# orybkin/video-gcp

Hardware: AMD Instinct MI355X
Metric: predicted frames/sec, 64x64x3 seq_len=80 gcp_tree (posterior forward + all loss terms, model(inputs) and model.loss() of train.py:157-159, batch-stat BatchNorm) (higher is better)
Workload: dtype f32 (encoder / decoder convs and the tree GEMMs from 512 rows: split-f16 MFMA with f32 accumulate, f32-equivalent; everything else exact f32 MFMA)

## Files before the change

### video-gcp_amd/csrc/aux.hip

```cpp
#include "common.h"

namespace {

template <bool GAUSS>
__global__ void aux_sample_indices_kernel(const long long* __restrict__ end_ind, const float* __restrict__ u, const int B,
                                          const int temp_dist, long long* __restrict__ t0, long long* __restrict__ t1,
                                          long long* __restrict__ cs, long long* __restrict__ ce) {
    const int b = blockIdx.x * blockDim.x + threadIdx.x;
    if (b >= B) return;
    const long long e = end_ind[b];
    const double ed = (double)e;
    auto uni = [&](int k) { const double v = (double)u[k * B + b]; return GAUSS ? 0.5 * erfc(-v * 0.70710678118654752440) : v; };
    long long a = (long long)floor(uni(0) * (ed - temp_dist + 1));
    a = max(min(a, e - temp_dist), 0ll);
    long long d = (long long)floor(uni(1) * temp_dist);
    d = min(d, (long long)temp_dist - 1);
    long long s = (long long)floor(uni(2) * ed);
    s = min(s, e - 1);
    long long w = (long long)floor(uni(3) * (ed - (double)s));
    w = min(w, e - s - 1);
    t0[b] = a;
    t1[b] = min(a + 1 + d, max(e, 0ll));
    cs[b] = s;
    ce[b] = s + 1 + w;
}

__global__ void aux_index_rows_kernel(const long long* __restrict__ t0, const long long* __restrict__ t1,
                                      const long long* __restrict__ cs, const long long* __restrict__ ce, const int B, const int T,
                                      const int Wd, int* __restrict__ rows) {
    const int b = blockIdx.x * blockDim.x + threadIdx.x;
    if (b >= B) return;
    rows[b] = b * T + (int)t0[b];
    rows[B + b] = b * Wd + (int)t1[b];
    rows[2 * B + b] = b * Wd + (int)cs[b];
    rows[3 * B + b] = b * Wd + (int)ce[b];
}

template <int VEC>
__global__ void __launch_bounds__(256) path_cost_rows_kernel(const float* __restrict__ x, const long long* __restrict__ cs,
                                                             const long long* __restrict__ ce, const int T, const int rows,
                                                             const int row_len, float* __restrict__ partial) {
    const int lane = threadIdx.x & 63;
    const int row = blockIdx.x * 4 + (threadIdx.x >> 6);
    const int b = blockIdx.y;
    if (row >= rows) return;
    const int s = (int)cs[b], e = (int)ce[b];
    const size_t frame = (size_t)rows * row_len;
    const float* p = x + ((size_t)b * T + s) * frame + (size_t)row * row_len;
    float acc = 0.f;
    for (int t = s; t < e; ++t) {
        float d2 = 0.f;
        for (int c = lane * VEC; c < row_len; c += 64 * VEC) {
#pragma unroll
            for (int v = 0; v < VEC; ++v) {
                if (c + v < row_len) {
                    const float d = p[frame + c + v] - p[c + v];
                    d2 = fmaf(d, d, d2);
                }
            }
        }
        for (int o = 32; o > 0; o >>= 1) d2 += __shfl_xor(d2, o);
        acc += sqrtf(d2);
        p += frame;
    }
    if (lane == 0) partial[(size_t)b * rows + row] = acc;
}

__global__ void __launch_bounds__(256) path_cost_finish_kernel(const float* __restrict__ partial, const int rows,
                                                               float* __restrict__ out) {
    __shared__ float red[256];
    const int b = blockIdx.x;
    float v = 0.f;
    for (int i = threadIdx.x; i < rows; i += 256) v += partial[(size_t)b * rows + i];
    red[threadIdx.x] = v;
    __syncthreads();
    for (int s = 128; s > 0; s >>= 1) {
        if (threadIdx.x < s) red[threadIdx.x] += red[threadIdx.x + s];
        __syncthreads();
    }
    if (threadIdx.x == 0) out[b] = red[0];
}

__global__ void __launch_bounds__(64) sample_length_kernel(const float* __restrict__ logits, const float* __restrict__ u,
                                                           const int T, const int min_len, long long* __restrict__ end_ind) {
    const int b = blockIdx.x, lane = threadIdx.x;
    const float* l = logits + (size_t)b * T;
    double m = -INFINITY;
    for (int t = lane; t < T; t += 64) m = fmax(m, (double)l[t]);
    for (int o = 32; o > 0; o >>= 1) m = fmax(m, __shfl_xor(m, o));
    double se = 0.0;
    for (int t = lane; t < T; t += 64) se += exp((double)l[t] - m);
    for (int o = 32; o > 0; o >>= 1) se += __shfl_xor(se, o);
    if (lane == 0) {
        const double target = (double)u[b];
        double c = 0.0;
        int idx = 0;
        for (int t = 0; t < T; ++t) {
            c += exp((double)l[t] - m) / se;
            if (c <= target) idx = t + 1;
        }
        idx = min(idx, T - 1);
        end_ind[b] = max(idx, min_len);
    }
}

}

#define STREAM() hipStream_t stream = reinterpret_cast<hipStream_t>(stream_)

extern "C" int gcpx_aux_sample_indices(const int64_t* end_ind, const float* u, int32_t B, int32_t temp_dist, int64_t* inv_t0,
                                       int64_t* inv_t1, int64_t* cost_start, int64_t* cost_end, void* stream_) {
    STREAM();
    GCPX_CHECK_ARG(end_ind && u && inv_t0 && inv_t1 && cost_start && cost_end && B > 0 && temp_dist >= 1, "bad arguments");
    hipLaunchKernelGGL(aux_sample_indices_kernel<false>, dim3((B + 63) / 64), dim3(64), 0, stream, (const long long*)end_ind, u, B, temp_dist,
                       (long long*)inv_t0, (long long*)inv_t1, (long long*)cost_start, (long long*)cost_end);
    GCPX_CHECK_LAUNCH();
    return GCPX_OK;
}

extern "C" int gcpx_aux_sample_indices_gauss(const int64_t* end_ind, const float* n, int32_t B, int32_t temp_dist, int64_t* inv_t0,
                                             int64_t* inv_t1, int64_t* cost_start, int64_t* cost_end, void* stream_) {
    STREAM();
    GCPX_CHECK_ARG(end_ind && n && inv_t0 && inv_t1 && cost_start && cost_end && B > 0 && temp_dist >= 1, "bad arguments");
    hipLaunchKernelGGL(aux_sample_indices_kernel<true>, dim3((B + 63) / 64), dim3(64), 0, stream, (const long long*)end_ind, n, B, temp_dist,
                       (long long*)inv_t0, (long long*)inv_t1, (long long*)cost_start, (long long*)cost_end);
    GCPX_CHECK_LAUNCH();
    return GCPX_OK;
}

extern "C" int gcpx_aux_index_rows(const int64_t* inv_t0, const int64_t* inv_t1, const int64_t* cost_start, const int64_t* cost_end,
                                   int32_t B, int32_t T, int32_t Wd, int32_t* rows, void* stream_) {
    STREAM();
    GCPX_CHECK_ARG(inv_t0 && inv_t1 && cost_start && cost_end && rows && B > 0 && T > 0 && Wd > 0, "bad arguments");
    hipLaunchKernelGGL(aux_index_rows_kernel, dim3((B + 63) / 64), dim3(64), 0, stream, (const long long*)inv_t0, (const long long*)inv_t1,
                       (const long long*)cost_start, (const long long*)cost_end, B, T, Wd, rows);
    GCPX_CHECK_LAUNCH();
    return GCPX_OK;
}

extern "C" int gcpx_path_cost(const float* x, const int64_t* start_idx, const int64_t* end_idx, int32_t B, int32_t T, int32_t rows,
                              int32_t row_len, float* partial, float* out, void* stream_) {
    STREAM();
    GCPX_CHECK_ARG(x && start_idx && end_idx && partial && out && B > 0 && T > 1 && rows > 0 && row_len > 0, "bad arguments");
    hipLaunchKernelGGL(path_cost_rows_kernel<1>, dim3((rows + 3) / 4, B), dim3(256), 0, stream, x, (const long long*)start_idx,
                       (const long long*)end_idx, T, rows, row_len, partial);
    hipLaunchKernelGGL(path_cost_finish_kernel, dim3(B), dim3(256), 0, stream, partial, rows, out);
    GCPX_CHECK_LAUNCH();
    return GCPX_OK;
}

extern "C" int gcpx_sample_length(const float* logits, const float* u, int32_t B, int32_t T, int32_t min_len, int64_t* end_ind,
                                  void* stream_) {
    STREAM();
    GCPX_CHECK_ARG(logits && u && end_ind && B > 0 && T > 0 && min_len >= 0 && min_len < T, "bad arguments");
    hipLaunchKernelGGL(sample_length_kernel, dim3(B), dim3(64), 0, stream, logits, u, T, min_len, (long long*)end_ind);
    GCPX_CHECK_LAUNCH();
    return GCPX_OK;
}
```

### video-gcp_amd/csrc/misc.hip

```cpp
#include "common.h"

#include <cstdarg>
#include <cstdio>

static thread_local char g_err[512] = "";

void gcpx_set_error(const char* fmt, ...) {
    va_list ap;
    va_start(ap, fmt);
    vsnprintf(g_err, sizeof(g_err), fmt, ap);
    va_end(ap);
}

extern "C" const char* gcpx_last_error(void) { return g_err; }
extern "C" int gcpx_version(void) { return GCPX_VERSION; }

namespace {

__global__ void __launch_bounds__(256) bn_finalize_kernel(const float* __restrict__ partial, const int n_partial,
                                                          const int pitch, const int C, const double count,
                                                          const float* __restrict__ gamma,
                                                          const float* __restrict__ beta, const float eps,
                                                          float* __restrict__ scale, float* __restrict__ shift,
                                                          float* running_mean, float* running_var,
// ... 51 lines not shown
#pragma unroll
    for (int r = 0; r < 10; ++r) {
        const unsigned hi0 = __umulhi(0xD2511F53u, c.x), lo0 = 0xD2511F53u * c.x;
        const unsigned hi1 = __umulhi(0xCD9E8D57u, c.z), lo1 = 0xCD9E8D57u * c.z;
        c = make_uint4(hi1 ^ c.y ^ k.x, lo1, hi0 ^ c.w ^ k.y, lo0);
        k.x += 0x9E3779B9u; k.y += 0xBB67AE85u;
    }
    return c;
}

__global__ void __launch_bounds__(256) randn_kernel(float* __restrict__ out, const long long n, const unsigned long long* __restrict__ state) {
    const unsigned long long seed = state[0], ctr = state[1] + (unsigned long long)blockIdx.x * 256 + threadIdx.x;
    const long long i = ((long long)blockIdx.x * 256 + threadIdx.x) * 4;
    if (i >= n) return;
    const uint4 r = philox4x32_10(make_uint4((unsigned)ctr, (unsigned)(ctr >> 32), 0u, 0u), make_uint2((unsigned)seed, (unsigned)(seed >> 32)));
    const float u0 = ((r.x >> 8) + 1u) * 5.9604644775390625e-8f, u1 = (r.y >> 8) * 5.9604644775390625e-8f;
    const float u2 = ((r.z >> 8) + 1u) * 5.9604644775390625e-8f, u3 = (r.w >> 8) * 5.9604644775390625e-8f;
    const float ra = sqrtf(-2.f * __logf(u0)), rb = sqrtf(-2.f * __logf(u2));
    float sa, ca, sb, cb;
    __sincosf(6.283185307179586f * u1, &sa, &ca);
    __sincosf(6.283185307179586f * u3, &sb, &cb);
    const float v[4] = {ra * ca, ra * sa, rb * cb, rb * sb};
    if (i + 3 < n) {
        *reinterpret_cast<float4*>(out + i) = make_float4(v[0], v[1], v[2], v[3]);
    } else {
        for (int k = 0; k < 4 && i + k < n; ++k) out[i + k] = v[k];
    }
}

__global__ void rng_advance_kernel(unsigned long long* state, const unsigned long long inc) { state[1] += inc; }

__global__ void bn_fold_kernel(const float* __restrict__ rm, const float* __restrict__ rv,
                               const float* __restrict__ gamma, const float* __restrict__ beta, const float eps,
                               const int C, float* __restrict__ scale, float* __restrict__ shift) {
    const int c = blockIdx.x * blockDim.x + threadIdx.x;
    if (c < C) {
        const float sc = gamma[c] / sqrtf(rv[c] + eps);
        scale[c] = sc;
        shift[c] = beta[c] - rm[c] * sc;
    }
}

__device__ __forceinline__ long long trunc_mid(long long tl, long long tr) {
    const long long s = tl + tr;
    return s >= 0 ? s / 2 : -((-s) / 2);
}

__global__ void __launch_bounds__(256) balanced_binding_kernel(const int64_t* __restrict__ end_ind, const int B,
                                                               const int L, const int T, int32_t* __restrict__ node_t,
                                                               int32_t* __restrict__ leave,
                                                               int32_t* __restrict__ frame2node,
                                                               int32_t* __restrict__ etilde_row,
                                                               int32_t* __restrict__ seq_len,
                                                               int32_t* __restrict__ node2row) {
    const int b = blockIdx.x;
    const int N = (1 << L) - 1;
    const long long end = end_ind[b];
    const int root = (N - 1) / 2;
    for (int t = threadIdx.x; t < T; t += blockDim.x) frame2node[(size_t)b * T + t] = root;
    if (threadIdx.x == 0) seq_len[b] = (int32_t)(end + 1);
    __syncthreads();
    for (int p = threadIdx.x; p < N; p += blockDim.x) {
        const int tz = __ffs(p + 1) - 1;
        const int l = L - 1 - tz;
        const int jn = (p + 1) >> (tz + 1);
        long long tl = -1, tr = end + 1, t = 0;
        for (int k = 0; k <= l; ++k) {
            t = trunc_mid(tl, tr);
            if (k == l) break;
            if ((jn >> (l - 1 - k)) & 1) tl = t; else tr = t;
        }
        const int keep = !(t == tl || t == tr);
        node_t[(size_t)b * N + p] = (int32_t)t;
        leave[(size_t)b * N + p] = keep;
        if (keep && t >= 0 && t < T) frame2node[(size_t)b * T + t] = p;
        if (node2row) node2row[(size_t)b * N + p] = (keep && t >= 0 && t < T) ? (int32_t)(b * T + t) : -1;
        if (etilde_row) {
            long long tc = t < 0 ? 0 : (t >= T ? T - 1 : t);
            etilde_row[(size_t)B * ((1 << l) - 1) + (size_t)b * (1 << l) + jn] = (int32_t)(b * T + tc);
        }
    }
}

__global__ void compact_index_kernel(const int32_t* __restrict__ leave, const int B, const int N, const int T,
                                     int32_t* __restrict__ dst) {
    const int b = blockIdx.x * blockDim.x + threadIdx.x;
    if (b >= B) return;
    int k = 0;
    for (int p = 0; p < N; ++p)
        if (leave[(size_t)b * N + p]) {
            if (k < T) dst[(size_t)b * T + k] = p;
            ++k;
        }
    for (; k < T; ++k) dst[(size_t)b * T + k] = -1;
}

__global__ void __launch_bounds__(256) gather_rows_kernel(const float* __restrict__ src, const int32_t* __restrict__ idx,
                                                          float* __restrict__ out, const int T, const int N,
                                                          const int idx_offset, const long long row4, const int32_t* __restrict__ skip) {
    const int bt = blockIdx.x;
    const int b = bt / T;
    if (skip && skip[bt] >= 0) return;
    const int i = idx[bt];
    float4* o = reinterpret_cast<float4*>(out) + (size_t)bt * row4;
    if (i < 0) {
        for (long long k = threadIdx.x; k < row4; k += blockDim.x) o[k] = make_float4(0.f, 0.f, 0.f, 0.f);
    } else {
        const float4* s = reinterpret_cast<const float4*>(src) + ((size_t)b * N + i + idx_offset) * row4;
        for (long long k = threadIdx.x; k < row4; k += blockDim.x) o[k] = s[k];
    }
}

__global__ void seq_pairs_kernel(const float* __restrict__ lat, const int32_t* __restrict__ lengths,
                                 const float* __restrict__ goal, float* __restrict__ nxt, const int T, const int nz4) {
    const int it = blockIdx.x;
    const int i = it / T, t = it % T;
    const int len = lengths[i];
    const float4* src;
    if (t + 1 < len) src = reinterpret_cast<const float4*>(lat) + ((size_t)i * T + t + 1) * nz4;
    else if (goal) src = reinterpret_cast<const float4*>(goal) + (size_t)i * nz4;
    else src = reinterpret_cast<const float4*>(lat) + ((size_t)i * T + (len > 0 ? len - 1 : 0)) * nz4;
    float4* dst = reinterpret_cast<float4*>(nxt) + (size_t)it * nz4;
    for (int k = threadIdx.x; k < nz4; k += blockDim.x) dst[k] = src[k];
}

__global__ void __launch_bounds__(256) copy_rows_kernel(const float* __restrict__ src, float* __restrict__ dst,
                                                        const int rows, const long long row4, const long long sbr,
                                                        const long long dbr) {
    const int b = blockIdx.x / rows, r = blockIdx.x % rows;
    const float4* s = reinterpret_cast<const float4*>(src) + ((size_t)b * sbr + r) * row4;
    float4* d = reinterpret_cast<float4*>(dst) + ((size_t)b * dbr + r) * row4;
    for (long long k = threadIdx.x; k < row4; k += blockDim.x) d[k] = s[k];
}

__global__ void gauss_sample_kernel(const float* __restrict__ muls, const long long mb, const long long mr,
                                    const float* __restrict__ eps, const long long eb, const long long er,
                                    float* __restrict__ z, const long long zb, const long long zr, const int M,
                                    const int rpb, const int nz) {
    const int i = blockIdx.x * blockDim.x + threadIdx.x;
    if (i >= M * nz) return;
    const int r = i / nz, d = i % nz;
    const int b = r / rpb, j = r % rpb;
    const float* m = muls + (size_t)b * mb + (size_t)j * mr;
    z[(size_t)b * zb + (size_t)j * zr + d] = m[d] + expf(m[nz + d]) * eps[(size_t)b * eb + (size_t)j * er + d];
}

__global__ void seq_index_kernel(const int64_t* __restrict__ end_ind, const int B, const int T, int32_t* __restrict__ idx,
                                 int32_t* __restrict__ seq_len) {
    const int i = blockIdx.x * blockDim.x + threadIdx.x;
    if (i >= B * T) return;
    const int b = i / T, t = i % T;
    const long long e = end_ind[b];
    idx[i] = (t <= e) ? t : -1;
    if (t == 0) seq_len[b] = (int32_t)(e + 1);
}

__global__ void masked_row_sum_kernel(const float* __restrict__ vals, const int32_t* __restrict__ lengths,
                                      float* __restrict__ out, const int n, const int T) {
    const int i = blockIdx.x * blockDim.x + threadIdx.x;
    if (i >= n) return;
    float s = 0.f;
    const int len = min(lengths[i], T);
    for (int t = 0; t < len; ++t) s += vals[(size_t)i * T + t];
    out[i] = s;
}

__global__ void __launch_bounds__(256) rollout_cost_kernel(const float* __restrict__ x, const long long ld, const int32_t* __restrict__ lengths,
                                                           const float* __restrict__ goal, const long long goal_stride, float* __restrict__ out,
                                                           const int T, const int D, const int kind, const int dense, const float final_w) {
    extern __shared__ float steps[];
    const int i = blockIdx.x, lane = threadIdx.x & 63, wave = threadIdx.x >> 6;
    const int len = min(lengths[i], T);
    const float* xi = x + (size_t)i * T * ld;
    const float* g = goal + (size_t)i * goal_stride;
    for (int t = wave; t < len; t += 4) {
        float s = 0.f;
        if (kind == 2) {
// ... 59 lines not shown
                       (long long)mr, eps, (long long)eb, (long long)er, z, (long long)zb, (long long)zr, M, rpb, nz);
    GCPX_CHECK_LAUNCH();
    return GCPX_OK;
}

extern "C" int gcpx_seq_index(const int64_t* end_ind, int32_t B, int32_t T, int32_t* idx, int32_t* seq_len, void* stream_) {
    hipStream_t stream = reinterpret_cast<hipStream_t>(stream_);
    GCPX_CHECK_ARG(end_ind && idx && seq_len && B > 0 && T > 0, "null pointer / bad sizes");
    hipLaunchKernelGGL(seq_index_kernel, dim3((B * T + 255) / 256), dim3(256), 0, stream, end_ind, B, T, idx, seq_len);
    GCPX_CHECK_LAUNCH();
    return GCPX_OK;
}

extern "C" int gcpx_fill_zero(void* ptr, int64_t nbytes, void* stream_) {
    GCPX_CHECK_ARG(ptr && nbytes > 0, "null pointer / bad size");
    hipError_t e = hipMemsetAsync(ptr, 0, (size_t)nbytes, reinterpret_cast<hipStream_t>(stream_));
    if (e != hipSuccess) {
        gcpx_set_error("gcpx_fill_zero: %s", hipGetErrorString(e));
        return GCPX_ERR_HIP;
    }
    return GCPX_OK;
}

extern "C" int gcpx_masked_row_sum(const float* vals, const int32_t* lengths, float* out, int32_t n, int32_t T,
                                   void* stream_) {
    hipStream_t stream = reinterpret_cast<hipStream_t>(stream_);
    GCPX_CHECK_ARG(vals && lengths && out && n > 0 && T > 0, "null pointer / bad sizes");
    hipLaunchKernelGGL(masked_row_sum_kernel, dim3((n + 63) / 64), dim3(64), 0, stream, vals, lengths, out, n, T);
    GCPX_CHECK_LAUNCH();
    return GCPX_OK;
}

extern "C" int gcpx_bn_finalize(const float* partial, int32_t n_partial, int32_t pitch, int32_t C, double count,
                                const float* gamma, const float* beta, float eps, float* scale, float* shift,
                                float* running_mean, float* running_var, float momentum, float* mean_out,
                                float* rstd_out, void* stream_) {
    hipStream_t stream = reinterpret_cast<hipStream_t>(stream_);
    GCPX_CHECK_ARG(partial && gamma && beta && scale && shift, "null pointer");
    GCPX_CHECK_ARG((mean_out == nullptr) == (rstd_out == nullptr), "mean_out and rstd_out go together");
    GCPX_CHECK_ARG(n_partial > 0 && C > 0 && pitch >= C && pitch % C == 0 && count > 0, "bad sizes");
    hipLaunchKernelGGL(bn_finalize_kernel, dim3(C), dim3(256), 0, stream, partial, n_partial, pitch, C, count, gamma,
                       beta, eps, scale, shift, running_mean, running_var, momentum, mean_out, rstd_out);
    GCPX_CHECK_LAUNCH();
    return GCPX_OK;
}

extern "C" int gcpx_randn(float* out, int64_t n, uint64_t* state, void* stream_) {
    hipStream_t stream = reinterpret_cast<hipStream_t>(stream_);
    GCPX_CHECK_ARG(out && state && n > 0 && (reinterpret_cast<uintptr_t>(out) & 15) == 0, "null pointer / n <= 0 / out not 16-byte aligned");
    const long long threads = (n + 3) / 4;
    const unsigned blocks = (unsigned)((threads + 255) / 256);
    hipLaunchKernelGGL(randn_kernel, dim3(blocks), dim3(256), 0, stream, out, (long long)n, reinterpret_cast<const unsigned long long*>(state));
    hipLaunchKernelGGL(rng_advance_kernel, dim3(1), dim3(1), 0, stream, reinterpret_cast<unsigned long long*>(state), (unsigned long long)blocks * 256);
    GCPX_CHECK_LAUNCH();
    return GCPX_OK;
}

extern "C" int gcpx_bn_fold(const float* running_mean, const float* running_var, const float* gamma,
                            const float* beta, float eps, int32_t C, float* scale, float* shift, void* stream_) {
    hipStream_t stream = reinterpret_cast<hipStream_t>(stream_);
    GCPX_CHECK_ARG(running_mean && running_var && gamma && beta && scale && shift && C > 0, "null pointer / C <= 0");
    hipLaunchKernelGGL(bn_fold_kernel, dim3((C + 63) / 64), dim3(64), 0, stream, running_mean, running_var, gamma, beta,
                       eps, C, scale, shift);
    GCPX_CHECK_LAUNCH();
    return GCPX_OK;
}

extern "C" int gcpx_balanced_binding(const int64_t* end_ind, int32_t B, int32_t L, int32_t T, int32_t* node_t,
                                     int32_t* leave, int32_t* frame2node, int32_t* etilde_row, int32_t* seq_len,
                                     int32_t* node2row, void* stream_) {
    hipStream_t stream = reinterpret_cast<hipStream_t>(stream_);
    GCPX_CHECK_ARG(end_ind && node_t && leave && frame2node && seq_len, "null pointer");
    GCPX_CHECK_ARG(B > 0 && L > 0 && L < 20 && T > 0, "bad sizes");
    hipLaunchKernelGGL(balanced_binding_kernel, dim3(B), dim3(256), 0, stream, end_ind, B, L, T, node_t, leave,
                       frame2node, etilde_row, seq_len, node2row);
    GCPX_CHECK_LAUNCH();
    return GCPX_OK;
}

extern "C" int gcpx_compact_index(const int32_t* leave, int32_t B, int32_t N, int32_t T, int32_t* dst_idx,
                                  void* stream_) {
    hipStream_t stream = reinterpret_cast<hipStream_t>(stream_);
    GCPX_CHECK_ARG(leave && dst_idx && B > 0 && N > 0 && T > 0, "null pointer / bad sizes");
    hipLaunchKernelGGL(compact_index_kernel, dim3((B + 63) / 64), dim3(64), 0, stream, leave, B, N, T, dst_idx);
    GCPX_CHECK_LAUNCH();
    return GCPX_OK;
}

extern "C" int gcpx_gather_rows(const float* src, const int32_t* idx, float* out, int32_t B, int32_t T, int32_t N,
                                int32_t idx_offset, int64_t row_floats, void* stream_) {
    hipStream_t stream = reinterpret_cast<hipStream_t>(stream_);
    GCPX_CHECK_ARG(src && idx && out && B > 0 && T > 0 && N > 0, "null pointer / bad sizes");
    GCPX_CHECK_ARG(row_floats > 0 && row_floats % 4 == 0, "row_floats must be a positive multiple of 4");
    hipLaunchKernelGGL(gather_rows_kernel, dim3(B * T), dim3(256), 0, stream, src, idx, out, T, N,
                       idx_offset, (long long)(row_floats / 4), static_cast<const int32_t*>(nullptr));
    GCPX_CHECK_LAUNCH();
    return GCPX_OK;
}

extern "C" int gcpx_gather_rows_rest(const float* src, const int32_t* idx, float* out, int32_t B, int32_t T, int32_t N, int32_t idx_offset,
                                     int64_t row_floats, const int32_t* written, void* stream_) {
    hipStream_t stream = reinterpret_cast<hipStream_t>(stream_);
    GCPX_CHECK_ARG(src && idx && out && written && B > 0 && T > 0 && N > 0, "null pointer / bad sizes");
    GCPX_CHECK_ARG(row_floats > 0 && row_floats % 4 == 0, "row_floats must be a positive multiple of 4");
    hipLaunchKernelGGL(gather_rows_kernel, dim3(B * T), dim3(256), 0, stream, src, idx, out, T, N,
                       idx_offset, (long long)(row_floats / 4), written);
    GCPX_CHECK_LAUNCH();
    return GCPX_OK;
}

#define GCPX_HIP(call)                                                            \
    do {                                                                          \
        hipError_t e_ = (call);                                                   \
        if (e_ != hipSuccess) {                                                   \
            gcpx_set_error("%s: %s failed: %s", __func__, #call, hipGetErrorString(e_)); \
            return GCPX_ERR_HIP;                                                  \
        }                                                                         \
    } while (0)

extern "C" int gcpx_graph_begin(void* stream) {
    GCPX_HIP(hipStreamBeginCapture(reinterpret_cast<hipStream_t>(stream), hipStreamCaptureModeThreadLocal));
    return GCPX_OK;
}

extern "C" int gcpx_graph_end(void* stream, void** graph_exec) {
    GCPX_CHECK_ARG(graph_exec != nullptr, "graph_exec is NULL");
    hipGraph_t graph = nullptr;
    GCPX_HIP(hipStreamEndCapture(reinterpret_cast<hipStream_t>(stream), &graph));
    hipGraphExec_t exec = nullptr;
    hipError_t e = hipGraphInstantiate(&exec, graph, nullptr, nullptr, 0);
    (void)hipGraphDestroy(graph);
    if (e != hipSuccess) {
        gcpx_set_error("gcpx_graph_end: hipGraphInstantiate failed: %s", hipGetErrorString(e));
        return GCPX_ERR_HIP;
    }
    *graph_exec = exec;
    return GCPX_OK;
}

extern "C" int gcpx_graph_launch(void* graph_exec, void* stream) {
    GCPX_HIP(hipGraphLaunch(reinterpret_cast<hipGraphExec_t>(graph_exec), reinterpret_cast<hipStream_t>(stream)));
    return GCPX_OK;
}

extern "C" int gcpx_graph_destroy(void* graph_exec) {
    GCPX_HIP(hipGraphExecDestroy(reinterpret_cast<hipGraphExec_t>(graph_exec)));
    return GCPX_OK;
}

extern "C" int gcpx_stream_create(void** stream) {
    GCPX_CHECK_ARG(stream != nullptr, "stream is NULL");
    hipStream_t s;
    GCPX_HIP(hipStreamCreateWithFlags(&s, hipStreamNonBlocking));
    *stream = s;
    return GCPX_OK;
}

extern "C" int gcpx_stream_create_priority(void** stream, int level) {
    GCPX_CHECK_ARG(stream != nullptr, "stream is NULL");
    int least = 0, greatest = 0;
    GCPX_HIP(hipDeviceGetStreamPriorityRange(&least, &greatest));
    const int prio = level < 0 ? greatest : (level > 0 ? least : (least + greatest) / 2);
    hipStream_t s;
    GCPX_HIP(hipStreamCreateWithPriority(&s, hipStreamNonBlocking, prio));
    *stream = s;
    return GCPX_OK;
}
// ... 44 lines not shown
```

### video-gcp_amd/forward_plan.py

```python
import ctypes as C
import os
from contextlib import contextmanager

import torch

from . import packing as pk
from . import runtime as rt
from .hparams import GCPHParams
from .params import init_params, encoder_layers, encoder_skip_layers, decoder_layers
from .plan_ops import _Plan, _addr, N_LANES


class ForwardPlanMixin:

    def _plan_encoder(self, plan, tag, x_ptr, F, out_ptr, out_ob, out_orow, out_rpb):
        hp, P, lib = self._hp, self.pk, self.lib
        G = lib.gcpx_conv4x4s2_grid()
        S = hp.img_sz
        skip_idx = encoder_skip_layers(hp)
        skips = {}
        a0 = self._buf(f"{tag}.a0", (F, S // 2, S // 2, hp.ngf))
        enc_rec = dict(F=F, x_ptr=x_ptr, a0=a0, r={}, out=(out_ptr, out_ob, out_orow, out_rpb))
        plan.rec[f"enc:{tag}"] = enc_rec
        plan.add(f"enc.input:{tag}", lib.gcpx_conv4x4s2_image, x_ptr, P["enc.input.w"].data_ptr(),
# ... 74 lines not shown
        plan.rec["dec"] = dict(F=F, rpb=rpb, e_src=e_src, d0=d0, blocks=[], skips=skips)
        nrb = lib.gcpx_gemm_row_blocks(F, 16 * ctop)
        st = self._buf("dec.st0", (nrb, 2, 16 * ctop)) if self.training else None
        self._gemm(plan, "dec.input", [e_src], F, 16 * ctop, rpb, P["dec.input.w"], P["dec.input.b"], out=d0.data_ptr(),
                   ob=rpb * 16 * ctop, orow=16 * ctop, stats=st)
        sc, sh = self._bn(plan, "dec.bn0", "decoder.net.input.norm", ctop, st, nrb, 16 * ctop, F * 16)
        prev = (d0.data_ptr(), ctop, 1, sc, sh, rt.ACT_LRELU)
        res = 4
        for name, c_prev, c_skip, skip_idx, cout in decoder_layers(hp):
            srcs = [prev]
            if skip_idx >= 0:
                t, C_, ssc, ssh, sact = skips[skip_idx]
                assert C_ == c_skip and t.shape[1] == res
                srcs.append((t.data_ptr(), C_, rpb, ssc, ssh, sact))
            o = self._buf(f"dec.{name}", (F, 2 * res, 2 * res, cout))
            cpad = (cout + 15) // 16 * 16
            hoist = (skip_idx >= 0 and rpb > 1 and F % rpb == 0 and self.split_f16 and cout in (32, 64) and c_prev % 32 == 0 and
                     c_skip % 32 == 0 and f"dec.{name}" in self.pk_split and "fold" not in self.pk_split[f"dec.{name}"] and
                     os.environ.get("GCPX_NO_SKIP_HOIST") is None)
            addend = None
            if hoist:
                addend = self._buf(f"dec.{name}.skip", (F // rpb, 2 * res, 2 * res, cout))
                t, C_, ssc, ssh, sact = skips[skip_idx]
                zb = self._buf(f"dec.{name}.zero_bias", (cpad,), zero=True)
                a_s = self._conv_args([(t.data_ptr(), C_, 1, ssc, ssh, sact)], F // rpb, res, res, 2 * res, 2 * res, cout, cout,
                                      P[f"dec.{name}.w"], zb, addend, upsample=1)
                self._set_split(a_s, f"dec.{name}")
                a_s.wpk_split = a_s.wpk_split + (c_prev // 32) * 9 * (cpad // 16) * 2048
                plan.keep.append(a_s)
                plan.add(f"dec.{name}.skip", lib.gcpx_conv3x3, C.byref(a_s))
                srcs_main = [prev]
            else:
                srcs_main = srcs
            a = self._conv_args(srcs_main, F, res, res, 2 * res, 2 * res, cout, cout, P[f"dec.{name}.w"], P[f"dec.{name}.b"],
                                o, upsample=1, stats=(o if self.training else None))
            if hoist:
                a.addend, a.addend_frame_div = addend.data_ptr(), rpb
            self._set_split(a, f"dec.{name}")
            Gl = lib.gcpx_conv3x3_grid(C.byref(a))
            assert Gl > 0, rt.lib().gcpx_last_error()
            st = self._buf(f"dec.st.{name}", (Gl, 2, cpad)) if self.training else None
            a.stats_partial = st.data_ptr() if st is not None else None
            plan.keep.append(a)
            plan.add(f"dec.{name}", lib.gcpx_conv3x3, C.byref(a))
            plan.rec["dec"]["blocks"].append(dict(name=name, srcs=srcs, out=o, res_in=res, cout=cout, c_prev=c_prev, c_skip=c_skip,
                                                  skip_idx=skip_idx))
            res *= 2
            sc, sh = self._bn(plan, f"dec.bn.{name}", f"decoder.net.{name}.norm", cout, st, Gl, cpad, F * res * res)
            prev = (o.data_ptr(), cout, 1, sc, sh, rt.ACT_LRELU)
        assert res == hp.img_sz
        return prev

    def _build_plan(self, key, tin):
        hp, P, lib = self._hp, self.pk, self.lib
        B, has_traj, has_z, sample_prior, phase = key[0], key[1], key[2], key[3], key[4]
        pred_len = key[9]
        train_aux = has_traj and phase == "train" and not sample_prior
        L, T, N = hp.hierarchy_levels, hp.max_seq_len, hp.n_nodes
        nz, nv, H, SD = hp.nz_enc, hp.nz_vae, hp.nz_mid_lstm, hp.lstm_state_dim
        PS = 2 ** L + 1
        plan = _Plan(lib)
        G = lib.gcpx_conv_grid()
        def plan_aux_indices():
            AUXK = ("inv_t0", "inv_t1", "cost_start_idx", "cost_end_idx")
            plan.add("aux_sample_indices", lib.gcpx_aux_sample_indices_gauss, tin["end_ind"].data_ptr(), tin["aux_n"].data_ptr(), B,
                     hp.inv_mdl_temp_dist, *[tin[k].data_ptr() for k in AUXK])
        if "aux_n" in tin and pred_len:
            plan_aux_indices()

        E = self._buf("E", (B, PS, nz))
        Hid = self._buf("Hid", (B, PS, SD))
        Z = self._buf("Z", (B, PS, nv))
        PZ = self._buf("PZ", (B, PS, 2 * nv))
        QZ = self._buf("QZ", (B, PS, 2 * nv))
        node_t = self._buf("node_t", (B, N), torch.int32)
        leave = self._buf("leave", (B, N), torch.int32)
        f2n = self._buf("frame2node", (B, T), torch.int32)
        etrow = self._buf("etilde_row", (B * N,), torch.int32)
        seq_len = self._buf("seq_len", (B,), torch.int32)
        kept_idx = self._buf("kept_idx", (B, T), torch.int32)
        node2row = self._buf("node2row", (B, N), torch.int32)

        adaptive, attentive = hp.adaptive, hp.attentive_inference
        if adaptive:
            kept_idx = self._buf("kept_idx", (B, N), torch.int32)
        def plan_bookkeeping():
            if not adaptive:
                plan.add("balanced_binding", lib.gcpx_balanced_binding, tin["end_ind"].data_ptr(), B, L, T, node_t.data_ptr(),
                         leave.data_ptr(), f2n.data_ptr(), etrow.data_ptr(), seq_len.data_ptr(), node2row.data_ptr())
                plan.add("compact_index", lib.gcpx_compact_index, leave.data_ptr(), B, N, T, kept_idx.data_ptr())
                r2f = self._buf("row2frame", (B * T,), torch.int32)
                if self._head_grad_fused(key) or self._rows_direct(key):
                    plan.add("row2frame", lib.gcpx_index_inverse, node2row.data_ptr(), B * N, r2f.data_ptr(), B * T)
                if self._head_grad_fused(key):
                    S_ = hp.img_sz
                    dMD = self._buf("bw.dMD", (B * T, S_, S_, self._head_pitch))
                    plan.add("zero_unmapped", lib.gcpx_zero_unmapped_rows, dMD.data_ptr(), S_ * S_ * self._head_pitch, r2f.data_ptr(), B * T)

        enc_traj = inf_enc = None
        plan.fork([1, 2])
        traj_first = os.environ.get("GCPX_ENC_ORDER") != "small_first"
        def plan_traj_encoder():
            nonlocal enc_traj, inf_enc
            plan.lane = 0
            if has_traj:
                enc_traj = self._buf("enc_traj", (B * T, nz))
                self._plan_encoder(plan, "traj", tin["traj_seq"].data_ptr(), B * T, enc_traj.data_ptr(), T * nz, nz, T)
                if hp.seq_enc == "none":
                    inf_enc = enc_traj
                else:
                    inf_enc = self._buf("inf_enc_seq", (B * T, nz))
                    self._plan_seq_encoder(plan, "seq", "inf_encoder", enc_traj, inf_enc, B)
                if attentive:
                    dk = hp.nz_attn_key
                    n_mod = L if hp.untied_layers else 1
                    if hp.seq_enc == "none":
                        kenc = enc_traj
                    else:
                        kenc = self._buf("inf_key_enc", (B * T, nz))
                        self._plan_seq_encoder(plan, "kseq", "inf_key_encoder.0", enc_traj, kenc, B)
                    keys = self._buf("inf_enc_key_seq", (B * T, dk))
                    dense = lambda t, w: self._rowsrc(t.data_ptr(), 0, w, w)
                    self._gemm(plan, "kseq.key", [dense(kenc, nz)], B * T, dk, B * T, P["kseq.key.w"], P["kseq.key.b"],
                               out=keys.data_ptr(), ob=0, orow=dk)
                    Kp = self._buf("attn.K", (n_mod, B * T, dk))
                    Vp = self._buf("attn.V", (n_mod, B * T, nz))
                    self._gemm(plan, "attn.k_proj", [dense(keys, dk)], B * T, dk, B * T, P["attn.k_proj.w"], P["attn.k_proj.b"],
                               out=Kp.data_ptr(), ob=0, orow=dk, batch=(n_mod, 0, P["attn.k_proj.w"][0].numel(), dk, B * T * dk))
                    self._gemm(plan, "attn.v_proj", [dense(inf_enc, nz)], B * T, nz, B * T, P["attn.v_proj.w"], P["attn.v_proj.b"],
                               out=Vp.data_ptr(), ob=0, orow=nz, batch=(n_mod, 0, P["attn.v_proj.w"][0].numel(), nz, B * T * nz))
                    plan.rec["attn_kv"] = dict(Kp=Kp, Vp=Vp, keys=keys, kenc=kenc, n_mod=n_mod)

        if traj_first:
            plan_traj_encoder()
        plan.lane = 1
        if "rng_all" in tin:
            plan.add("randn", lib.gcpx_randn, tin["rng_all"].data_ptr(), tin["rng_all"].numel(), self._buf("rng_state", (2,), torch.int64).data_ptr())
            if "aux_n" in tin and not pred_len:
                plan.wait(2, 1)
        skips = self._plan_encoder(plan, "I0", tin["I_0"].data_ptr(), B, _addr(E), PS * nz, 0, 1)
        plan.lane = 2
        if not pred_len:
            if "aux_n" in tin:
                plan_aux_indices()
            plan_bookkeeping()
        if hp.attach_cost_mdl and hp.run_cost_mdl and train_aux and self._has_aux_training:
            gt = self._buf("cost_target", (B,))
            rows = hp.input_nc * hp.img_sz
            plan.add("path_cost", lib.gcpx_path_cost, tin["traj_seq"].data_ptr(), tin["cost_start_idx"].data_ptr(),
                     tin["cost_end_idx"].data_ptr(), B, T, rows, hp.img_sz, self._buf("cost_partial", (B, rows)).data_ptr(), gt.data_ptr())
        self._plan_encoder(plan, "Ig", tin["I_g"].data_ptr(), B, _addr(E, 2 ** L * nz), PS * nz, 0, 1)
        outs = {}
        e0 = lambda: self._rowsrc(_addr(E), PS * nz, 0, nz)
        eg = lambda: self._rowsrc(_addr(E, 2 ** L * nz), PS * nz, 0, nz)
        if hp.regress_length and not pred_len:
            plan.wait(2, 1)
            logits = self._buf("seq_len_logits", (B, T))
            self._mlp(plan, "length_pred", P["length_pred"], [e0(), eg()], B, 1, out=logits.data_ptr(), ob=T, orow=0)
            outs["seq_len_logits"] = logits
        if not traj_first:
            plan_traj_encoder()
        plan.lane = 0
        plan.join([1, 2])

        if hp.regress_length and pred_len:
            logits = self._buf("seq_len_logits", (B, T))
            self._mlp(plan, "length_pred", P["length_pred"], [e0(), eg()], B, 1, out=logits.data_ptr(), ob=T, orow=0)
            outs["seq_len_logits"] = logits
            plan.add("sample_length", lib.gcpx_sample_length, logits.data_ptr(), tin["len_u"].data_ptr(), B, T, 2, tin["end_ind"].data_ptr())
            plan_bookkeeping()

        side_merge = False
        for l in range(L):
            W = P[f"tree{l if hp.untied_layers else 0}"]
            s = 2 ** (L - 1 - l)
            n = 2 ** l
            M = B * n
            nodeoff = lambda w: s * w
            el = lambda: self._rowsrc(_addr(E), PS * nz, 2 * s * nz, nz)
            er = lambda: self._rowsrc(_addr(E, 2 * s * nz), PS * nz, 2 * s * nz, nz)
            pz_out = (_addr(PZ, nodeoff(2 * nv)), PS * 2 * nv, 2 * s * 2 * nv)
            z_map = (_addr(Z, nodeoff(nv)), PS * nv, 2 * s * nv)
            nl = hp.n_lstm_layers
            merged = self._buf(f"merged{l}", (M, 2 * nl * H))

            def plan_merge(lv=l, group=None):
                s_, n_ = 2 ** (L - 1 - lv), 2 ** lv
                Wl = P[f"tree{lv if hp.untied_layers else 0}"]
                mg = self._buf(f"merged{lv}", (B * n_, 2 * nl * H))
                if hp.tree_lstm == "sum":
                    for side, mode in ((0, 0), (2 * s_ * SD, 1)):
                        plan.add(f"merge{lv}.{mode}", lib.gcpx_rows_strided, _addr(mg), n_ * SD, SD, _addr(Hid, side), PS * SD, 2 * s_ * SD,
                                 B, n_, SD, mode)
                    return
                if hp.tree_lstm == "linear":
                    h1 = self._rowsrc(_addr(Hid), PS * SD, 2 * s_ * SD, SD)
                    h2 = self._rowsrc(_addr(Hid, 2 * s_ * SD), PS * SD, 2 * s_ * SD, SD)
                    self._gemm(plan, f"merge{lv}", [h1, h2], B * n_, SD, n_, Wl["proj.w"], Wl["proj.b"], out=_addr(mg), ob=n_ * SD, orow=SD,
                               group=group)
                    return
                h1 = self._rowsrc(_addr(Hid), PS * SD, 2 * s_ * SD, H)
                h2 = self._rowsrc(_addr(Hid, 2 * s_ * SD), PS * SD, 2 * s_ * SD, H)
                self._gemm(plan, f"merge{lv}", [h1, h2], B * n_, H, n_, Wl["proj.w"], Wl["proj.b"], out=_addr(mg),
                           ob=n_ * 2 * nl * H, orow=2 * nl * H, batch=(2 * nl, H, Wl["proj.w"][0].numel(), H, H), group=group)

            merge_with_predictors = not has_z and not sample_prior and hp.tree_lstm not in ("sum", "")
            if has_z:
                g = (_addr(tin["z"], (s - 1) * nv), N * nv, 2 * s * nv) + z_map
                self._mlp(plan, f"prior{l}", W["prior"], [el(), er()], M, n, out=pz_out[0], ob=pz_out[1], orow=pz_out[2], gauss=g)
            elif sample_prior:
                g = (_addr(tin["eps"], (n - 1) * nv), N * nv, nv) + z_map
                self._mlp(plan, f"prior{l}", W["prior"], [el(), er()], M, n, out=pz_out[0], ob=pz_out[1], orow=pz_out[2], gauss=g)
            else:
                pq = []
                self._mlp(plan, f"prior{l}", W["prior"], [el(), er()], M, n, out=pz_out[0], ob=pz_out[1], orow=pz_out[2], group=pq)
                if attentive:
                    et = self._plan_attention(plan, l, W, el(), er(), M, n, B, plan.rec["attn_kv"]["Kp"], plan.rec["attn_kv"]["Vp"], tin)
                else:
                    et = self._rowsrc(inf_enc.data_ptr(), 0, nz, nz, rowidx=etrow[B * (n - 1):])
                g = (_addr(tin["eps"], (n - 1) * nv), N * nv, nv) + z_map
                self._mlp(plan, f"posterior{l}", W["q"], [el(), er(), et], M, n, out=_addr(QZ, nodeoff(2 * nv)),
                          ob=PS * 2 * nv, orow=2 * s * 2 * nv, gauss=g, group=pq)
                mg = []
                if l > 0 and merge_with_predictors and not side_merge:
                    plan_merge(l, group=mg)
                self._mlp_group(plan, f"prior+posterior{l}", pq, gemm=(mg[0] if mg else None))
                if side_merge:
                    plan.join([1])
                    side_merge = False
            zs = lambda: self._rowsrc(z_map[0], z_map[1], z_map[2], nv)
            if not hp.tree_lstm:
                srcs = [el(), er(), zs()] + ([e0(), eg()] if hp.context_every_step else [])
                self._mlp(plan, f"subgoal{l}", W["sg"], srcs, M, n, out=_addr(E, nodeoff(nz)), ob=PS * nz, orow=2 * s * nz, tanh=True)
                continue
            if l == 0:
                if hp.lstm_init == "zero":
                    for slot in (0, 2 ** L):
                        plan.add(f"lstm_init.zero{slot}", lib.gcpx_rows_strided, _addr(Hid, slot * SD), PS * SD, 0, self._zero_row(SD).data_ptr(),
                                 0, 0, B, 1, SD, 0)
                else:
                    self._mlp(plan, "lstm_init", W["init"], [el(), er(), zs()], M, n, out=_addr(Hid), ob=PS * SD, orow=0,
                              oblk=2 ** L * SD, out_split=SD)
                plan_merge()
            x = self._buf(f"x{l}.0", (M, H))
            srcs = [el(), er(), zs()] + ([e0(), eg()] if hp.context_every_step else [])
            fused = "lstm0f.w" in W and not self.save_for_backward
            if not fused:
                self._gemm(plan, f"embed{l}", srcs, M, H, n, W["embed.w"], W["embed.b"], out=x.data_ptr(), ob=n * H, orow=H)
            for i in range(nl):
                xn = self._buf(f"x{l}.{i + 1}", (M, H))
                xs = self._rowsrc(x.data_ptr(), n * H, H, H)
                hs = self._rowsrc(_addr(merged, 2 * i * H), n * 2 * nl * H, 2 * nl * H, H)
                lstm = (_addr(merged, (2 * i + 1) * H), 2 * nl * H, _addr(Hid, nodeoff(SD) + 2 * i * H),
                        _addr(Hid, nodeoff(SD) + (2 * i + 1) * H), PS * SD, 2 * s * SD, xn.data_ptr())
                if i == 0 and fused:
                    self._gemm(plan, f"lstm{l}.0", srcs + [hs], M, 4 * H, n, W["lstm0f.w"], W["lstm0f.b"], epi=rt.EPI_LSTM, lstm=lstm)
                else:
                    self._gemm(plan, f"lstm{l}.{i}", [xs, hs], M, 4 * H, n, W[f"lstm{i}.w"], W[f"lstm{i}.b"],
                               epi=rt.EPI_LSTM, lstm=lstm)
                x = xn
            g = []
            self._gemm(plan, f"out{l}", [self._rowsrc(x.data_ptr(), n * H, H, H)], M, nz, n, W["out.w"], W["out.b"],
                       out=_addr(E, nodeoff(nz)), ob=PS * nz, orow=2 * s * nz, group=g)
            if l + 1 < L and not merge_with_predictors:
                plan_merge(l + 1, group=g)
            self._gemm_group(plan, f"out{l}+merge{l + 1}" if len(g) > 1 else f"out{l}", g)
            if (l + 1 < L and merge_with_predictors and hp.tree_lstm == "split_linear" and B * 2 ** (l + 1) >= self._merge_side_rows):
                plan.fork([1])
                plan.lane = 1
                plan_merge(l + 1)
                plan.lane = 0
                side_merge = True

        F = B * N
        matching = adaptive and has_traj and phase == "train"

        heads = []

        def plan_aux(idx, Wd):
            mes = self._buf("model_enc_seq", (B, Wd, nz))
            plan.add("gather.model_enc_seq", lib.gcpx_gather_rows, E.data_ptr(), idx.data_ptr(), mes.data_ptr(), B, Wd, PS, 1, nz)
            outs["model_enc_seq_padded"] = mes
            if hp.run_state_regressor:
                rs = self._buf("regressed_state", (B, Wd, hp.state_dim))
                self._mlp(plan, "state_regressor", P["state_regressor"], [self._rowsrc(mes.data_ptr(), Wd * nz, nz, nz)],
                          B * Wd, Wd, out=rs.data_ptr(), ob=Wd * hp.state_dim, orow=hp.state_dim, group=heads)
                outs["regressed_state_padded"] = rs
            if hp.attach_inv_mdl and phase == "train" and (sample_prior or hp.train_inv_mdl_full_seq or not has_traj):
                act = self._buf("actions", (B, Wd - 1, hp.n_actions))
                first = enc_traj if has_traj else mes
                s0 = self._rowsrc(first.data_ptr(), (T if has_traj else Wd) * nz, nz, nz)
                s1 = self._rowsrc(_addr(mes, nz), Wd * nz, nz, nz)
                self._mlp(plan, "inv_mdl", P["inv_mdl"], [s0, s1], B * (Wd - 1), Wd - 1, out=act.data_ptr(),
                          ob=(Wd - 1) * hp.n_actions, orow=hp.n_actions, group=heads)
                outs["actions_padded"] = act
            aux_rows = None
            if train_aux and ((hp.attach_inv_mdl and not hp.train_inv_mdl_full_seq) or (hp.attach_cost_mdl and hp.run_cost_mdl)):
                aux_rows = self._buf("aux_rows", (4, B), torch.int32)
                plan.add("aux_index_rows", lib.gcpx_aux_index_rows, tin["inv_t0"].data_ptr(), tin["inv_t1"].data_ptr(),
                         tin["cost_start_idx"].data_ptr(), tin["cost_end_idx"].data_ptr(), B, T, Wd, aux_rows.data_ptr())
                gather = lambda t, i: self._rowsrc(t.data_ptr(), 0, nz, nz, rowidx=aux_rows[i])
            if hp.attach_inv_mdl and train_aux and not hp.train_inv_mdl_full_seq:
                act = self._buf("actions_sampled", (B, hp.n_actions))
                self._mlp(plan, "inv_mdl", P["inv_mdl"], [gather(enc_traj, 0), gather(mes, 1)], B, B, out=act.data_ptr(), ob=0,
                          orow=hp.n_actions, group=heads)
                outs["actions_sampled"] = act
            if hp.attach_cost_mdl and hp.run_cost_mdl and train_aux:
                cost = self._buf("cost_pred", (B, 1))
                self._mlp(plan, "cost_mdl", P["cost_mdl"], [gather(mes, 2), gather(mes, 3)], B, B, out=cost.data_ptr(), ob=0, orow=1,
                          group=heads)
                outs["cost_pred"], outs["cost_target"] = cost, self._buf("cost_target", (B,))

        heads_lane = 0
        if heads_lane:
            plan.fork([1])
        plan.lane = heads_lane
        if adaptive:
            dist = self._buf("distances", (B, N - 1))
            self._mlp(plan, "distance", P["distance"], [self._rowsrc(_addr(E, nz), PS * nz, nz, nz),
                                                        self._rowsrc(_addr(E, 2 * nz), PS * nz, nz, nz)],
                      B * (N - 1), N - 1, out=dist.data_ptr(), ob=N - 1, orow=1)
            pruned_len = self._buf("pruned_len", (B,), torch.int32)
            plan.add("distance_prune", lib.gcpx_distance_prune, dist.data_ptr(), C.c_float(hp.learned_pruning_threshold), None, B, N,
                     leave.data_ptr(), kept_idx.data_ptr(), pruned_len.data_ptr(), None)
            outs["distances"], outs["pruned_len"] = dist, pruned_len
            if not matching:
                plan_aux(kept_idx, N)
                outs["aux_len"] = pruned_len
        else:
            plan_aux(kept_idx, T)
            exist = self._buf("existence", (B, N))
            self._mlp(plan, "existence", P["existence"], [self._rowsrc(_addr(E, nz), PS * nz, nz, nz)], F, N,
                      out=exist.data_ptr(), ob=N, orow=1, group=heads)
            outs["existence"] = exist
        if heads:
            self._mlp_group(plan, "heads", heads)
            heads.clear()
        plan.lane = 0

        def kl_args(kl_b, batch=()):
            return (_addr(QZ, 2 * nv), _addr(PZ, 2 * nv)) + batch + (N, nv, PS * 2 * nv, 2 * nv, C.c_float(hp.free_nats), None, 0, kl_b.data_ptr())

        def loss_args():
            kl_b = self._buf("kl_b", (B,))
            la = rt.LossArgs()
            la.nll_bt, la.pad_mask, la.kl_b = self._buf("nll_bt", (B, T)).data_ptr(), tin["pad_mask"].data_ptr(), kl_b.data_ptr()
            la.len_logits = outs["seq_len_logits"].data_ptr() if "seq_len_logits" in outs else None
            la.end_ind = tin["end_ind"].data_ptr()
            if adaptive:
                la.existence, la.leave = outs["distances"].data_ptr(), outs["distance_target"].data_ptr()
            else:
                la.existence, la.leave = outs["existence"].data_ptr(), leave.data_ptr()
            if "regressed_state_padded" in outs and "traj_seq_states" in tin:
                la.regressed_state, la.state_target = outs["regressed_state_padded"].data_ptr(), tin["traj_seq_states"].data_ptr()
            la.seq_len = seq_len.data_ptr()
            if "actions_sampled" in outs and "actions" in tin:
                la.action_pred, la.action_seq, la.inv_t0 = outs["actions_sampled"].data_ptr(), tin["actions"].data_ptr(), tin["inv_t0"].data_ptr()
                la.n_actions, la.w_action = hp.n_actions, hp.action_rec_weight
            if "cost_pred" in outs:
                la.cost_pred, la.cost_target, la.w_cost = outs["cost_pred"].data_ptr(), outs["cost_target"].data_ptr(), 1.0
            loss_out = self._buf("losses", (16,), zero=True)
            la.out, la.B, la.T, la.N, la.state_dim = loss_out.data_ptr(), B, T, (N - 1 if adaptive else N), hp.state_dim
            la.w_rec, la.w_kl, la.w_len, la.w_exist, la.w_state = hp.dense_img_rec_weight, hp.kl_weight, hp.length_pred_weight, 1.0, 1.0
            if self._kl_w is not None:
                la.w_kl_dev = self._kl_w.data_ptr()
            la.total_div = float(T * hp.input_nc * hp.img_sz * hp.img_sz)
            plan.keep.append(la)
            return la, kl_b

        decode, with_loss = key[8], key[7]
        loss_pre = None
        if with_loss and not adaptive:
            loss_pre = loss_args()
            plan.add("loss.pre", lib.gcpx_loss_pre, C.byref(loss_pre[0]), *kl_args(loss_pre[1]))
        if decode:
            F = B * N
            S = hp.img_sz
            prev = self._plan_decoder_features(plan, self._rowsrc(_addr(E, nz), PS * nz, nz, nz), F, N, skips)
            images = self._buf("images_df", (B, N, hp.input_nc, S, S))
            distr = matched_distr = None
            with_loss = key[7]
            dlm = hp.decoder_distribution == "discrete_logistic_mixture"
            head_out, row_map = None, None
            fused_nll = None
            if dlm:
                mode = rt.HEAD_DLM_MEAN
                if self.materialize_distr or (adaptive and self.save_for_backward and with_loss):
                    mode, distr = rt.HEAD_DLM_BOTH, self._buf("distr_df", (B, N, S, S, self._head_pitch))
                    head_out = distr
                elif self._head_grad_fused(key):
                    mode, row_map = rt.HEAD_DLM_NLL_GRAD, node2row
                    head_out = self._buf("bw.dMD", (B * T, S, S, self._head_pitch))
                    fused_nll = self._buf("nll_partial", ((S // 4) * (S // 16), B * T), zero=True)
                    plan.rec["nll_bwd_fused"] = plan.rec["head_grad_fused"] = True
                elif with_loss and not adaptive and not self.save_for_backward and self._head_nll_fusable():
                    mode, row_map = rt.HEAD_DLM_NLL, node2row
# ... 128 lines not shown
```

Baseline: 487,700.

## Overlap goal encoder and bookkeeping with tree via early event, speed aux kernels

Reorders the side lane so the goal encoder and balanced binding run first and signal the main lane through an event. Aux indices, compact index, aux row indexing and path cost then continue on the side lane, overlapping with the tree computation, and are joined later before the heads. The path cost kernel is rewritten to keep per-lane register values across time steps, so each frame is loaded once and loads are unrolled. compact_index becomes a wave-parallel ballot/popcount compaction instead of one thread per batch item. This adds event-ordering complexity and the risk of a race if aux_rows is used before its producer finishes.

```diff
diff --git a/video-gcp_amd/csrc/aux.hip b/video-gcp_amd/csrc/aux.hip
--- a/video-gcp_amd/csrc/aux.hip
+++ b/video-gcp_amd/csrc/aux.hip
@@ -36,7 +36,15 @@
     rows[3 * B + b] = b * Wd + (int)ce[b];
 }
 
-template <int VEC>
+constexpr int PATH_COST_U = 8;
+constexpr int PATH_COST_MAX_NCH = 2;
+
+__device__ __forceinline__ float wave_sum(float v) {
+    for (int o = 32; o > 0; o >>= 1) v += __shfl_xor(v, o);
+    return v;
+}
+
+template <int NCH, int U>
 __global__ void __launch_bounds__(256) path_cost_rows_kernel(const float* __restrict__ x, const long long* __restrict__ cs,
                                                              const long long* __restrict__ ce, const int T, const int rows,
                                                              const int row_len, float* __restrict__ partial) {
@@ -47,20 +55,65 @@
     const int s = (int)cs[b], e = (int)ce[b];
     const size_t frame = (size_t)rows * row_len;
     const float* p = x + ((size_t)b * T + s) * frame + (size_t)row * row_len;
+    auto load = [&](const float* q, float (&v)[NCH]) {
+#pragma unroll
+        for (int j = 0; j < NCH; ++j) {
+            const int c = lane + 64 * j;
+            const float f = q[min(c, row_len - 1)];
+            v[j] = c < row_len ? f : 0.f;
+        }
+    };
+    auto step = [&](float (&cur)[NCH], const float (&nxt)[NCH]) {
+        float d2 = 0.f;
+#pragma unroll
+        for (int j = 0; j < NCH; ++j) {
+            const float d = nxt[j] - cur[j];
+            d2 = fmaf(d, d, d2);
+            cur[j] = nxt[j];
+        }
+        return sqrtf(wave_sum(d2));
+    };
+    float acc = 0.f;
+    if (e > s) {
+        float cur[NCH];
+        load(p, cur);
+        int t = s;
+        for (; t + U <= e; t += U) {
+            float nxt[U][NCH];
+#pragma unroll
+            for (int u = 0; u < U; ++u) load(p + (size_t)(u + 1) * frame, nxt[u]);
+#pragma unroll
+            for (int u = 0; u < U; ++u) acc += step(cur, nxt[u]);
+            p += (size_t)U * frame;
+        }
+        for (; t < e; ++t) {
+            float nxt[NCH];
+            load(p + frame, nxt);
+            acc += step(cur, nxt);
+            p += frame;
+        }
+    }
+    if (lane == 0) partial[(size_t)b * rows + row] = acc;
+}
+
+__global__ void __launch_bounds__(256) path_cost_rows_loop_kernel(const float* __restrict__ x, const long long* __restrict__ cs,
+                                                                  const long long* __restrict__ ce, const int T, const int rows,
+                                                                  const int row_len, float* __restrict__ partial) {
+    const int lane = threadIdx.x & 63;
+    const int row = blockIdx.x * 4 + (threadIdx.x >> 6);
+    const int b = blockIdx.y;
+    if (row >= rows) return;
+    const int s = (int)cs[b], e = (int)ce[b];
+    const size_t frame = (size_t)rows * row_len;
+    const float* p = x + ((size_t)b * T + s) * frame + (size_t)row * row_len;
     float acc = 0.f;
     for (int t = s; t < e; ++t) {
         float d2 = 0.f;
-        for (int c = lane * VEC; c < row_len; c += 64 * VEC) {
-#pragma unroll
-            for (int v = 0; v < VEC; ++v) {
-                if (c + v < row_len) {
-                    const float d = p[frame + c + v] - p[c + v];
-                    d2 = fmaf(d, d, d2);
-                }
-            }
-        }
-        for (int o = 32; o > 0; o >>= 1) d2 += __shfl_xor(d2, o);
-        acc += sqrtf(d2);
+        for (int c = lane; c < row_len; c += 64) {
+            const float d = p[frame + c] - p[c];
+            d2 = fmaf(d, d, d2);
+        }
+        acc += sqrtf(wave_sum(d2));
         p += frame;
     }
     if (lane == 0) partial[(size_t)b * rows + row] = acc;
@@ -142,8 +195,12 @@
                               int32_t row_len, float* partial, float* out, void* stream_) {
     STREAM();
     GCPX_CHECK_ARG(x && start_idx && end_idx && partial && out && B > 0 && T > 1 && rows > 0 && row_len > 0, "bad arguments");
-    hipLaunchKernelGGL(path_cost_rows_kernel<1>, dim3((rows + 3) / 4, B), dim3(256), 0, stream, x, (const long long*)start_idx,
-                       (const long long*)end_idx, T, rows, row_len, partial);
+    const dim3 grid((rows + 3) / 4, B);
+    static_assert(PATH_COST_MAX_NCH == 2, "one launch per NCH below");
+    auto rows_kernel = row_len <= 64 ? path_cost_rows_kernel<1, PATH_COST_U>
+                       : row_len <= 128 ? path_cost_rows_kernel<2, PATH_COST_U> : path_cost_rows_loop_kernel;
+    hipLaunchKernelGGL(rows_kernel, grid, dim3(256), 0, stream, x, (const long long*)start_idx, (const long long*)end_idx, T, rows,
+                       row_len, partial);
     hipLaunchKernelGGL(path_cost_finish_kernel, dim3(B), dim3(256), 0, stream, partial, rows, out);
     GCPX_CHECK_LAUNCH();
     return GCPX_OK;
diff --git a/video-gcp_amd/csrc/misc.hip b/video-gcp_amd/csrc/misc.hip
--- a/video-gcp_amd/csrc/misc.hip
+++ b/video-gcp_amd/csrc/misc.hip
@@ -157,17 +157,23 @@
     }
 }
 
-__global__ void compact_index_kernel(const int32_t* __restrict__ leave, const int B, const int N, const int T,
-                                     int32_t* __restrict__ dst) {
-    const int b = blockIdx.x * blockDim.x + threadIdx.x;
+__global__ void __launch_bounds__(256) compact_index_kernel(const int32_t* __restrict__ leave, const int B, const int N, const int T,
+                                                            int32_t* __restrict__ dst) {
+    const int lane = threadIdx.x & 63;
+    const int b = blockIdx.x * 4 + (threadIdx.x >> 6);
     if (b >= B) return;
-    int k = 0;
-    for (int p = 0; p < N; ++p)
-        if (leave[(size_t)b * N + p]) {
-            if (k < T) dst[(size_t)b * T + k] = p;
-            ++k;
-        }
-    for (; k < T; ++k) dst[(size_t)b * T + k] = -1;
+    const int32_t* lv = leave + (size_t)b * N;
+    int32_t* d = dst + (size_t)b * T;
+    int count = 0;
+    for (int p0 = 0; p0 < N; p0 += 64) {
+        const int p = p0 + lane;
+        const bool keep = p < N && lv[p] != 0;
+        const unsigned long long m = __ballot(keep);
+        const int rank = count + __popcll(m & ((1ull << lane) - 1ull));
+        if (keep && rank < T) d[rank] = p;
+        count += __popcll(m);
+    }
+    for (int k = count + lane; k < T; k += 64) d[k] = -1;
 }
 
 __global__ void __launch_bounds__(256) gather_rows_kernel(const float* __restrict__ src, const int32_t* __restrict__ idx,
@@ -393,7 +399,7 @@
                                   void* stream_) {
     hipStream_t stream = reinterpret_cast<hipStream_t>(stream_);
     GCPX_CHECK_ARG(leave && dst_idx && B > 0 && N > 0 && T > 0, "null pointer / bad sizes");
-    hipLaunchKernelGGL(compact_index_kernel, dim3((B + 63) / 64), dim3(64), 0, stream, leave, B, N, T, dst_idx);
+    hipLaunchKernelGGL(compact_index_kernel, dim3((B + 3) / 4), dim3(256), 0, stream, leave, B, N, T, dst_idx);
     GCPX_CHECK_LAUNCH();
     return GCPX_OK;
 }
diff --git a/video-gcp_amd/forward_plan.py b/video-gcp_amd/forward_plan.py
--- a/video-gcp_amd/forward_plan.py
+++ b/video-gcp_amd/forward_plan.py
@@ -180,12 +180,16 @@
         node2row = self._buf("node2row", (B, N), torch.int32)
 
         adaptive, attentive = hp.adaptive, hp.attentive_inference
+        tree_early = not pred_len and not adaptive and not self.save_for_backward
         if adaptive:
             kept_idx = self._buf("kept_idx", (B, N), torch.int32)
-        def plan_bookkeeping():
+        def plan_binding():
             if not adaptive:
                 plan.add("balanced_binding", lib.gcpx_balanced_binding, tin["end_ind"].data_ptr(), B, L, T, node_t.data_ptr(),
                          leave.data_ptr(), f2n.data_ptr(), etrow.data_ptr(), seq_len.data_ptr(), node2row.data_ptr())
+
+        def plan_bookkeeping_rest():
+            if not adaptive:
                 plan.add("compact_index", lib.gcpx_compact_index, leave.data_ptr(), B, N, T, kept_idx.data_ptr())
                 r2f = self._buf("row2frame", (B * T,), torch.int32)
                 if self._head_grad_fused(key) or self._rows_direct(key):
@@ -194,6 +198,20 @@
                     S_ = hp.img_sz
                     dMD = self._buf("bw.dMD", (B * T, S_, S_, self._head_pitch))
                     plan.add("zero_unmapped", lib.gcpx_zero_unmapped_rows, dMD.data_ptr(), S_ * S_ * self._head_pitch, r2f.data_ptr(), B * T)
+
+        def plan_bookkeeping():
+            plan_binding()
+            plan_bookkeeping_rest()
+
+        aux_rows_wanted = train_aux and ((hp.attach_inv_mdl and not hp.train_inv_mdl_full_seq) or (hp.attach_cost_mdl and hp.run_cost_mdl))
+        aux_rows_planned = []
+
+        def plan_aux_rows(Wd):
+            aux_rows = self._buf("aux_rows", (4, B), torch.int32)
+            plan.add("aux_index_rows", lib.gcpx_aux_index_rows, tin["inv_t0"].data_ptr(), tin["inv_t1"].data_ptr(),
+                     tin["cost_start_idx"].data_ptr(), tin["cost_end_idx"].data_ptr(), B, T, Wd, aux_rows.data_ptr())
+            aux_rows_planned.append(Wd)
+            return aux_rows
 
         enc_traj = inf_enc = None
         plan.fork([1, 2])
@@ -232,22 +250,47 @@
         if traj_first:
             plan_traj_encoder()
         plan.lane = 1
+        randn_done = None
         if "rng_all" in tin:
             plan.add("randn", lib.gcpx_randn, tin["rng_all"].data_ptr(), tin["rng_all"].numel(), self._buf("rng_state", (2,), torch.int64).data_ptr())
             if "aux_n" in tin and not pred_len:
-                plan.wait(2, 1)
+                if tree_early:
+                    randn_done = plan.record(1)
+                else:
+                    plan.wait(2, 1)
         skips = self._plan_encoder(plan, "I0", tin["I_0"].data_ptr(), B, _addr(E), PS * nz, 0, 1)
         plan.lane = 2
-        if not pred_len:
+
+        def plan_path_cost():
+            if hp.attach_cost_mdl and hp.run_cost_mdl and train_aux and self._has_aux_training:
+                gt = self._buf("cost_target", (B,))
+                rows = hp.input_nc * hp.img_sz
+                plan.add("path_cost", lib.gcpx_path_cost, tin["traj_seq"].data_ptr(), tin["cost_start_idx"].data_ptr(),
+                         tin["cost_end_idx"].data_ptr(), B, T, rows, hp.img_sz, self._buf("cost_partial", (B, rows)).data_ptr(), gt.data_ptr())
+
+        def plan_goal_encoder():
+            self._plan_encoder(plan, "Ig", tin["I_g"].data_ptr(), B, _addr(E, 2 ** L * nz), PS * nz, 0, 1)
+
+        tree_inputs_done = None
+        if tree_early:
+            plan_goal_encoder()
+            plan_binding()
+            tree_inputs_done = plan.record(2)
             if "aux_n" in tin:
+                if randn_done is not None:
+                    plan.await_event(2, randn_done)
                 plan_aux_indices()
-            plan_bookkeeping()
-        if hp.attach_cost_mdl and hp.run_cost_mdl and train_aux and self._has_aux_training:
-            gt = self._buf("cost_target", (B,))
-            rows = hp.input_nc * hp.img_sz
-            plan.add("path_cost", lib.gcpx_path_cost, tin["traj_seq"].data_ptr(), tin["cost_start_idx"].data_ptr(),
-                     tin["cost_end_idx"].data_ptr(), B, T, rows, hp.img_sz, self._buf("cost_partial", (B, rows)).data_ptr(), gt.data_ptr())
-        self._plan_encoder(plan, "Ig", tin["I_g"].data_ptr(), B, _addr(E, 2 ** L * nz), PS * nz, 0, 1)
+            if aux_rows_wanted:
+                plan_aux_rows(T)
+            plan_bookkeeping_rest()
+            plan_path_cost()
+        else:
+            if not pred_len:
+                if "aux_n" in tin:
+                    plan_aux_indices()
+                plan_bookkeeping()
+            plan_path_cost()
+            plan_goal_encoder()
         outs = {}
         e0 = lambda: self._rowsrc(_addr(E), PS * nz, 0, nz)
         eg = lambda: self._rowsrc(_addr(E, 2 ** L * nz), PS * nz, 0, nz)
@@ -259,7 +302,11 @@
         if not traj_first:
             plan_traj_encoder()
         plan.lane = 0
-        plan.join([1, 2])
+        if tree_early:
+            plan.join([1])
+            plan.await_event(0, tree_inputs_done)
+        else:
+            plan.join([1, 2])
 
         if hp.regress_length and pred_len:
             logits = self._buf("seq_len_logits", (B, T))
@@ -393,10 +440,8 @@
                           ob=(Wd - 1) * hp.n_actions, orow=hp.n_actions, group=heads)
                 outs["actions_padded"] = act
             aux_rows = None
-            if train_aux and ((hp.attach_inv_mdl and not hp.train_inv_mdl_full_seq) or (hp.attach_cost_mdl and hp.run_cost_mdl)):
-                aux_rows = self._buf("aux_rows", (4, B), torch.int32)
-                plan.add("aux_index_rows", lib.gcpx_aux_index_rows, tin["inv_t0"].data_ptr(), tin["inv_t1"].data_ptr(),
-                         tin["cost_start_idx"].data_ptr(), tin["cost_end_idx"].data_ptr(), B, T, Wd, aux_rows.data_ptr())
+            if aux_rows_wanted:
+                aux_rows = self._buf("aux_rows", (4, B), torch.int32) if Wd in aux_rows_planned else plan_aux_rows(Wd)
                 gather = lambda t, i: self._rowsrc(t.data_ptr(), 0, nz, nz, rowidx=aux_rows[i])
             if hp.attach_inv_mdl and train_aux and not hp.train_inv_mdl_full_seq:
                 act = self._buf("actions_sampled", (B, hp.n_actions))
@@ -410,6 +455,8 @@
                 outs["cost_pred"], outs["cost_target"] = cost, self._buf("cost_target", (B,))
 
         heads_lane = 0
+        if tree_early:
+            plan.join([2])
         if heads_lane:
             plan.fork([1])
         plan.lane = heads_lane
```

Measured after the change: 488,900, median of 6. Within noise of the previous version (+0.2%).
